# DrewSingletary/asif

Hardware: AMD Instinct MI355X
Metric: QP solves/sec (batched filter()) (higher is better)
Workload: dtype f64

## Files before the change

asif_amd/csrc/capi.hip:

```cpp
#include "asif_hip.h"
#include "launchers.hpp"
#include "multi_own.hpp"
#include <cmath>
#include <cstdlib>
#include <cstring>
#include <new>
#include <thread>
#include <vector>

using namespace asif;

struct asif_hip_ctx {
	int model, variant, device;
	asif_hip_options opts;
	asif_hip_solver solver;
	asif_hip_dims dims;
	DevOptions dev;
	double *d_in, *d_out;
	int32_t *d_rc;
	int64_t cap;
	double *s_rows;
	int64_t s_cap;
	int32_t *s_code;
	int64_t s_code_cap;
	double *s_ckpt;
	int64_t s_ckpt_cap;
	struct Realizable {
		asif_hip_realizable_options opts;
		RzDev dev;
		double *d_vertices, *d_normals, *d_facetRec, *d_table, *d_pointC;
		int32_t *d_fverts, *d_factive, *d_overflow;
	} *rz;
	struct RobustData {
		asif_hip_robust_data_options opts;
		RbDev dev;
		double *d_hp, *d_pointC;
	} *rb;
	double *d_learn;
	DevOptions::Learn learn;
	int32_t *r_rc;
	int64_t r_cap;
};

extern "C" int asif_hip_version(void) { return ASIF_HIP_VERSION; }

extern "C" const char *asif_hip_error_string(int code)
{
	switch (code) {
	case ASIF_HIP_OK: return "ok";
	case ASIF_HIP_EINVAL: return "invalid argument or unsupported model/variant pair";
	case ASIF_HIP_ENODEVICE: return "no usable HIP device (gfx950 required)";
	case ASIF_HIP_EUNSUPPORTED: return "no compiled kernel for this QP shape";
	default: return code > 0 ? hipGetErrorString((hipError_t)code) : "unknown error";
	}
}

extern "C" int asif_hip_device_count(void)
{
	int n = 0;
	if (hipGetDeviceCount(&n) != hipSuccess) return 0;
	return n;
}

extern "C" int asif_hip_default_options(int model, int variant, asif_hip_options *o)
{
	if (!o) return ASIF_HIP_EINVAL;
	std::memset(o, 0, sizeof(*o));
	o->relaxCost = 50.0;
	o->relaxLb = 5.0;
	o->relaxReachLb = 5.0;
	o->relaxTTS = 5.0;
	o->relaxMinOrtho = 5.0;
	o->backTrajHorizon = 1.0;
	o->backTrajExtend = 0.05;
	o->backTrajDt = 0.01;
	o->backTrajMinOrtho = 0.01;
	o->satSharpness = (variant == ASIF_HIP_EXPLICIT) ? 5.0 : 0.1;
	o->inf = 1e20;
	o->pMin = o->pMax = 1.0;
	o->backContDt = 0.01;
	o->n_debug = -1;
	o->npSSmax = -1;
	o->integrator = 0;
	o->backTrajAbsTol = 1.0e-6;
	o->backTrajRelTol = 1.0e-6;
	switch (model) {
	case ASIF_HIP_MODEL_DOUBLE_INTEGRATOR:
		o->lb[0] = -1.0;
		o->ub[0] = 1.0;
		break;
	case ASIF_HIP_MODEL_PLANAR_TWO_INPUT:
		o->lb[0] = o->lb[1] = -1.0;
		o->ub[0] = o->ub[1] = 1.0;
		break;
	case ASIF_HIP_MODEL_CART_PENDULUM:
		o->lb[0] = -4.0;
		o->ub[0] = 4.0;
		break;
	case ASIF_HIP_MODEL_INVERTED_PENDULUM:
		o->lb[0] = -1.5;
		o->ub[0] = 1.5;
		o->backTrajHorizon = 5.0;
		o->backTrajDt = 0.001;
		o->relaxReachLb = 5.0;
		o->relaxLb = 10.0;
		break;
	case ASIF_HIP_MODEL_SEGWAY:
		o->lb[0] = -20.0;
		o->ub[0] = 20.0;
		o->backTrajHorizon = 3.0;
		o->backTrajDt = 0.01;
		o->relaxCost = 10;
		o->relaxLb = 2.0;
		o->relaxTTS = 30.0;
		o->relaxMinOrtho = 60.0;
		o->backTrajMinOrtho = 0.001;
		break;
	case ASIF_HIP_MODEL_DOUBLE_INTEGRATOR_IMPLICIT:
		o->lb[0] = -1.0;
		o->ub[0] = 1.0;
		o->backTrajHorizon = 2.0;
		o->backTrajDt = 0.01;
		o->relaxReachLb = 5.0;
		o->relaxLb = 10.0;
		break;
	case ASIF_HIP_MODEL_DOUBLE_INTEGRATOR_TB:
		o->lb[0] = -1.0;
		o->ub[0] = 1.0;
		o->backTrajHorizon = 2.0;
		o->backTrajDt = 0.001;
		o->relaxLb = 10.0;
		o->relaxTTS = 5.0;
		o->relaxMinOrtho = 5.0;
		break;
	case ASIF_HIP_MODEL_INVERTED_PENDULUM_TB:
		o->lb[0] = -1.5;
		o->ub[0] = 1.5;
		o->backTrajHorizon = 11.0;
		o->backTrajDt = 0.001;
		o->relaxCost = 10.;
		o->relaxLb = 10.0;
		o->relaxTTS = 30.0;
		o->relaxMinOrtho = 60.0;
		o->backTrajMinOrtho = 0.001;
		break;
	case ASIF_HIP_MODEL_INVERTED_PENDULUM_ROBUST: {
		o->lb[0] = -1.5;
		o->ub[0] = 1.5;
		o->pMin = 0.8;
		o->pMax = 1.2;
		o->nHalfPlanes = 4;
		const double a = 1.0 / M_PI;
		const double hp[8] = {a, 0, -a, 0, 0, a, 0, -a};
		std::memcpy(o->halfPlanes, hp, sizeof(hp));
		break;
	}
	default:
		return ASIF_HIP_EINVAL;
	}
	return ASIF_HIP_OK;
}

extern "C" int asif_hip_default_solver(asif_hip_solver *s)
{
	if (!s) return ASIF_HIP_EINVAL;
	s->rho = 0.1;
	s->sigma = 1e-6;
	s->alpha = 1.6;
	s->eps_abs = 1e-8;
	s->eps_rel = 1e-8;
	s->eps_prim_inf = 1e-4;
	s->eps_dual_inf = 1e-4;
	s->adaptive_rho_tolerance = 5.0;
	s->max_iter = 4000;
	s->check_interval = 0;
	s->scaling_iters = 0;
	s->polish = 2;
	s->active_set_rounds = 12;
	s->refine_steps = 2;
	s->adaptive_rho = 1;
	s->lanes_per_qp = 0;
	s->presolve = 0;
	s->warm_start = 1;
	s->adaptive_rho_interval = 0;
	return ASIF_HIP_OK;
}

static double no_bound_value(double inf) { return inf > 1e30 ? 1e30 : inf; }

static int model_dims(int model, int variant, const asif_hip_options &o, asif_hip_dims &d, DevOptions &dev,
                      bool after_update = false)
{
	std::memset(&d, 0, sizeof(d));
	std::memset(&dev, 0, sizeof(dev));
// ... 448 lines not shown
	delete r;
}

static int rb_configure(asif_hip_ctx *c, const asif_hip_robust_data_options &o)
{
	asif_hip_ctx::RobustData *r = c->rb;
	RbDev &z = r->dev;
	int M = o.npSSmax;
	if (M < 0 || M > z.N) M = z.N;
	if (M < 1 || M > 8) return ASIF_HIP_EUNSUPPORTED;
	r->opts = o;
	z.npSSmax = M;
	z.relaxCost = o.relaxCost;
	z.relaxLb = o.relaxLb;
	z.inf = no_bound_value(o.inf);
	z.lb = o.lb[0];
	z.ub = o.ub[0];
	z.mMin = o.mMin;
	z.mMax = o.mMax;
	z.Klo = o.Klo;
	z.Khi = o.Khi;
	z.Flo = o.Flo;
	z.Fhi = o.Fhi;
	asif_hip_dims &d = c->dims;
	std::memset(&d, 0, sizeof(d));
	d.nx = 2;
	d.nu = 1;
	d.npSS = z.N;
	d.nv = 2 + 4 * M;
	d.nc = 3 * M;
	d.nrelax = 1;
	d.ndiag = M + 1;
	int rc = launch_robust_data_point(z, r->d_pointC, nullptr);
	if (rc) return rc;
	double pc[kRbPoint];
	hipError_t e = hipMemcpy(pc, r->d_pointC, sizeof(pc), hipMemcpyDeviceToHost);
	if (e != hipSuccess) return (int)e;
	return pc[kRbPoint - 1] != 0.0 ? ASIF_HIP_EUNSUPPORTED : ASIF_HIP_OK;
}

extern "C" int asif_hip_create_robust_data(asif_hip_ctx **out, int model, const double *halfPlanes, int32_t N,
                                           const asif_hip_robust_data_options *opts, const asif_hip_solver *solver,
                                           int device)
{
	if (!out) return ASIF_HIP_EINVAL;
	*out = nullptr;
	if (model != ASIF_HIP_MODEL_DOUBLE_INTEGRATOR_ROBUST || !halfPlanes || N < 1) return ASIF_HIP_EINVAL;
	asif_hip_robust_data_options o;
	if (opts) o = *opts;
	else asif_hip_default_robust_data_options(model, &o);
	int r = check_device(device);
	if (r) return r;
	hipError_t e = hipSetDevice(device);
	if (e != hipSuccess) return (int)e;
	asif_hip_ctx *c = new (std::nothrow) asif_hip_ctx();
	if (!c) return ASIF_HIP_EINVAL;
	std::memset(c, 0, sizeof(*c));
	c->model = model;
	c->variant = ASIF_HIP_ROBUST;
	c->device = device;
	if (solver) c->solver = *solver;
	else asif_hip_default_solver(&c->solver);
	c->rb = new (std::nothrow) asif_hip_ctx::RobustData();
	if (!c->rb) {
		delete c;
		return ASIF_HIP_EINVAL;
	}
	std::memset(c->rb, 0, sizeof(*c->rb));
	c->rb->dev.N = N;
	e = hipMalloc((void **)&c->rb->d_hp, sizeof(double) * 2 * N);
	if (e == hipSuccess) e = hipMalloc((void **)&c->rb->d_pointC, sizeof(double) * kRbPoint);
	if (e == hipSuccess) e = hipMemcpy(c->rb->d_hp, halfPlanes, sizeof(double) * 2 * N, hipMemcpyHostToDevice);
	c->rb->dev.hp = c->rb->d_hp;
	c->rb->dev.pointC = c->rb->d_pointC;
	r = (e == hipSuccess) ? rb_configure(c, o) : (int)e;
	if (r != ASIF_HIP_OK) {
		rb_free(c->rb);
		delete c;
		return r;
	}
	*out = c;
	return ASIF_HIP_OK;
}

extern "C" int asif_hip_update_robust_data_options(asif_hip_ctx *ctx, const asif_hip_robust_data_options *opts)
{
	if (!ctx || !opts || !ctx->rb) return ASIF_HIP_EINVAL;
	hipError_t e = hipSetDevice(ctx->device);
	if (e != hipSuccess) return (int)e;
	const asif_hip_robust_data_options keep = ctx->rb->opts;
	int r = rb_configure(ctx, *opts);
	if (r) (void)rb_configure(ctx, keep);
	return r;
}

extern "C" int asif_hip_destroy(asif_hip_ctx *ctx)
{
	if (!ctx) return ASIF_HIP_EINVAL;
	if (ctx->rz) {
		(void)hipSetDevice(ctx->device);
		rz_free(ctx->rz);
	}
	if (ctx->rb) {
		(void)hipSetDevice(ctx->device);
		rb_free(ctx->rb);
	}
	if (ctx->d_learn) {
		(void)hipSetDevice(ctx->device);
		(void)hipFree(ctx->d_learn);
	}
	if (ctx->r_rc) {
		(void)hipSetDevice(ctx->device);
		(void)hipFree(ctx->r_rc);
	}
	if (ctx->s_rows) {
		(void)hipSetDevice(ctx->device);
		(void)hipFree(ctx->s_rows);
	}
	if (ctx->s_code) {
		(void)hipSetDevice(ctx->device);
		(void)hipFree(ctx->s_code);
	}
	if (ctx->s_ckpt) {
		(void)hipSetDevice(ctx->device);
		(void)hipFree(ctx->s_ckpt);
	}
	if (ctx->d_in) {
		(void)hipSetDevice(ctx->device);
		(void)hipFree(ctx->d_in);
		(void)hipFree(ctx->d_out);
		(void)hipFree(ctx->d_rc);
	}
	delete ctx;
	return ASIF_HIP_OK;
}

extern "C" int asif_hip_get_dims(const asif_hip_ctx *ctx, asif_hip_dims *d)
{
	if (!ctx || !d) return ASIF_HIP_EINVAL;
	*d = ctx->dims;
	return ASIF_HIP_OK;
}

extern "C" int asif_hip_update_options(asif_hip_ctx *ctx, const asif_hip_options *opts)
{
	if (!ctx || !opts) return ASIF_HIP_EINVAL;
	asif_hip_dims d;
	DevOptions dev;
	int r = model_dims(ctx->model, ctx->variant, *opts, d, dev, true);
	if (r) return r;
	ctx->opts = *opts;
	ctx->dims = d;
	ctx->dev = dev;
	return ASIF_HIP_OK;
}

static int stage_rows(asif_hip_ctx *ctx, FilterArgs &a)
{
	const int64_t nA = (int64_t)ctx->dims.nc * ctx->dims.nv, nb = ctx->dims.nc;
	const int64_t need = (nA + nb) * a.ld;
	if (need > ctx->s_cap) {
		if (ctx->s_rows) (void)hipFree(ctx->s_rows);
		ctx->s_rows = nullptr;
		ctx->s_cap = 0;
		hipError_t e = hipMalloc((void **)&ctx->s_rows, sizeof(double) * need);
		if (e != hipSuccess) return (int)e;
		ctx->s_cap = need;
	}
	if (a.B > ctx->s_code_cap) {
		if (ctx->s_code) (void)hipFree(ctx->s_code);
		ctx->s_code = nullptr;
		ctx->s_code_cap = 0;
		hipError_t e = hipMalloc((void **)&ctx->s_code, sizeof(int32_t) * a.B);
		if (e != hipSuccess) return (int)e;
		ctx->s_code_cap = a.B;
	}
	a.A = ctx->s_rows;
	a.b = ctx->s_rows + nA * a.ld;
	a.code = ctx->s_code;
	return 0;
}

static int stage_ckpt(asif_hip_ctx *ctx, FilterArgs &a)
{
	const int64_t nz = ctx->dims.nx + ctx->dims.nx * ctx->dims.nx;
	int64_t need;
	switch (ctx->model) {
	case ASIF_HIP_MODEL_INVERTED_PENDULUM:
	case ASIF_HIP_MODEL_DOUBLE_INTEGRATOR_IMPLICIT:
	case ASIF_HIP_MODEL_INVERTED_PENDULUM_TB:
	case ASIF_HIP_MODEL_DOUBLE_INTEGRATOR_TB:
	case ASIF_HIP_MODEL_SEGWAY: need = (int64_t)ctx->dims.npBTSS * (nz + 2) * a.ld; break;
	default: return ASIF_HIP_EINVAL;
	}
	if (need > ctx->s_ckpt_cap) {
		if (ctx->s_ckpt) (void)hipFree(ctx->s_ckpt);
		ctx->s_ckpt = nullptr;
		ctx->s_ckpt_cap = 0;
		hipError_t e = hipMalloc((void **)&ctx->s_ckpt, sizeof(double) * need);
		if (e != hipSuccess) return (int)e;
		ctx->s_ckpt_cap = need;
	}
	a.ckpt = ctx->s_ckpt;
	return 0;
}

static int run_filter(asif_hip_ctx *ctx, FilterArgs a, bool assemble_only, hipStream_t stream)
{
	if (ctx->variant == ASIF_HIP_REALIZABLE)
		return ctx->rz ? launch_realizable(ctx->rz->dev, ctx->solver, a, assemble_only, stream) : ASIF_HIP_EINVAL;
	if (ctx->rb) return launch_robust_data(ctx->rb->dev, ctx->solver, a, assemble_only, stream);
	if (ctx->model == ASIF_HIP_MODEL_DOUBLE_INTEGRATOR && ctx->variant == ASIF_HIP_EXPLICIT)
		return launch_explicit_di(ctx->dev, ctx->solver, a, assemble_only, stream);
	if (ctx->model == ASIF_HIP_MODEL_PLANAR_TWO_INPUT && ctx->variant == ASIF_HIP_EXPLICIT)
		return launch_explicit_p2(ctx->dev, ctx->solver, a, assemble_only, stream);
	if (ctx->model == ASIF_HIP_MODEL_CART_PENDULUM && ctx->variant == ASIF_HIP_EXPLICIT)
		return launch_explicit_cp(ctx->dev, ctx->solver, a, assemble_only, stream);
	if (ctx->variant == ASIF_HIP_IMPLICIT_RB || (ctx->variant == ASIF_HIP_IMPLICIT && ctx->dev.useLearning)) {
		DevOptions dev = ctx->dev;
		if (dev.useLearning) {
			if (!ctx->d_learn) return ASIF_HIP_EINVAL;
			dev.learn = ctx->learn;
		}
		if (!assemble_only) {
			int r = stage_rows(ctx, a);
			if (r) return r;
		}
		if (int r = stage_ckpt(ctx, a)) return r;
		if (ctx->model == ASIF_HIP_MODEL_INVERTED_PENDULUM)
			return launch_implicit_ip(dev, ctx->solver, a, assemble_only, stream, true);
		if (ctx->model == ASIF_HIP_MODEL_DOUBLE_INTEGRATOR_IMPLICIT)
			return launch_implicit_di(dev, ctx->solver, a, assemble_only, stream, true);
		return ASIF_HIP_EINVAL;
	}
	if (ctx->model == ASIF_HIP_MODEL_INVERTED_PENDULUM && ctx->variant == ASIF_HIP_IMPLICIT) {
		if (!assemble_only) {
			int r = stage_rows(ctx, a);
			if (r) return r;
		}
		if (int r = stage_ckpt(ctx, a)) return r;
		return launch_implicit_ip(ctx->dev, ctx->solver, a, assemble_only, stream);
	}
	if (ctx->model == ASIF_HIP_MODEL_SEGWAY && ctx->variant == ASIF_HIP_IMPLICIT_TB) {
		if (!assemble_only) {
			int r = stage_rows(ctx, a);
			if (r) return r;
		}
		if (int r = stage_ckpt(ctx, a)) return r;
		return launch_tb_segway(ctx->dev, ctx->solver, a, assemble_only, stream);
	}
	if (ctx->model == ASIF_HIP_MODEL_DOUBLE_INTEGRATOR_IMPLICIT && ctx->variant == ASIF_HIP_IMPLICIT) {
		if (!assemble_only) {
			int r = stage_rows(ctx, a);
			if (r) return r;
		}
		if (int r = stage_ckpt(ctx, a)) return r;
		return launch_implicit_di(ctx->dev, ctx->solver, a, assemble_only, stream);
	}
	if (ctx->model == ASIF_HIP_MODEL_INVERTED_PENDULUM_TB && ctx->variant == ASIF_HIP_IMPLICIT_TB) {
		if (!assemble_only) {
			int r = stage_rows(ctx, a);
			if (r) return r;
		}
		if (int r = stage_ckpt(ctx, a)) return r;
		return launch_tb_pendulum(ctx->dev, ctx->solver, a, assemble_only, stream);
	}
	if (ctx->model == ASIF_HIP_MODEL_DOUBLE_INTEGRATOR_TB && ctx->variant == ASIF_HIP_IMPLICIT_TB) {
		if (!assemble_only) {
			int r = stage_rows(ctx, a);
			if (r) return r;
		}
		if (int r = stage_ckpt(ctx, a)) return r;
		return launch_tb_di(ctx->dev, ctx->solver, a, assemble_only, stream);
	}
	if (ctx->model == ASIF_HIP_MODEL_INVERTED_PENDULUM_ROBUST && ctx->variant == ASIF_HIP_ROBUST)
		return launch_robust_ip(ctx->dev, ctx->solver, a, assemble_only, stream);
	return ASIF_HIP_EINVAL;
}

extern "C" int asif_hip_filter_batch(asif_hip_ctx *ctx, int64_t B, int64_t ldx, const double *x, const double *udes,
                                     double *uact, double *relax, int32_t *rc, double *diag, void *stream)
{
	if (!ctx || B < 0 || ldx < B || (B > 0 && (!x || !udes || !uact || !relax || !rc))) return ASIF_HIP_EINVAL;
	if (B == 0) return ASIF_HIP_OK;
	hipError_t e = hipSetDevice(ctx->device);
	if (e != hipSuccess) return (int)e;
	FilterArgs a = {B, ldx, x, udes, uact, relax, rc, diag, ctx->dims.ndiag, nullptr, nullptr, nullptr};
	return run_filter(ctx, a, false, (hipStream_t)stream);
}

extern "C" int asif_hip_filter_batch_lie(asif_hip_ctx *ctx, int64_t B, int64_t ldx, const double *x, const double *udes,
                                         const double *lfh, const double *lgh, double *uact, double *relax, int32_t *rc,
                                         double *diag, void *stream)
{
	if (!ctx || B < 0 || ldx < B || (B > 0 && (!x || !udes || !lfh || !lgh || !uact || !relax || !rc)))
		return ASIF_HIP_EINVAL;
	if (ctx->variant != ASIF_HIP_EXPLICIT || ctx->rz || ctx->rb) return ASIF_HIP_EINVAL;
	if (B == 0) return ASIF_HIP_OK;
	hipError_t e = hipSetDevice(ctx->device);
	if (e != hipSuccess) return (int)e;
	FilterArgs a = {B, ldx, x, udes, uact, relax, rc, diag, ctx->dims.ndiag, nullptr, nullptr, nullptr, nullptr, lfh, lgh};
	return run_filter(ctx, a, false, (hipStream_t)stream);
}

static bool default_solver_mode(const asif_hip_solver &S, bool presolve_too = false)
{
	const bool light = S.polish == 2 || (presolve_too && S.presolve);
	return light && (S.lanes_per_qp == 0 || S.lanes_per_qp == 1);
}

extern "C" int asif_hip_filter_vjp_batch(asif_hip_ctx *ctx, int64_t B, int64_t ldx, const double *x, const double *udes,
                                         const double *lfh, const double *lgh, const double *guact, double *gudes,
                                         double *glfh, double *glgh, double *gx, int32_t *rc, void *stream)
{
	if (!ctx || B < 0 || ldx < B || (B > 0 && (!x || !udes || !guact || !gudes || !rc))) return ASIF_HIP_EINVAL;
	if ((lfh == nullptr) != (lgh == nullptr)) return ASIF_HIP_EINVAL;
	if (!lfh && (glfh || glgh || gx)) return ASIF_HIP_EINVAL;
	if (ctx->variant != ASIF_HIP_EXPLICIT || ctx->rz || ctx->rb) return ASIF_HIP_EUNSUPPORTED;
	if (!default_solver_mode(ctx->solver)) return ASIF_HIP_EUNSUPPORTED;
	if (B == 0) return ASIF_HIP_OK;
	hipError_t e = hipSetDevice(ctx->device);
	if (e != hipSuccess) return (int)e;
	const VjpArgs a = {B, ldx, x, udes, lfh, lgh, guact, gudes, glfh, glgh, gx, rc};
	if (ctx->model == ASIF_HIP_MODEL_DOUBLE_INTEGRATOR) return launch_explicit_vjp_di(ctx->dev, a, (hipStream_t)stream);
	if (ctx->model == ASIF_HIP_MODEL_PLANAR_TWO_INPUT) return launch_explicit_vjp_p2(ctx->dev, a, (hipStream_t)stream);
	if (ctx->model == ASIF_HIP_MODEL_CART_PENDULUM) return launch_explicit_vjp_cp(ctx->dev, a, (hipStream_t)stream);
	return ASIF_HIP_EUNSUPPORTED;
}

extern "C" int asif_hip_rollout_batch(asif_hip_ctx *ctx, int64_t B, int64_t ldx, int32_t T, double dt, double *x,
                                      const double *udes, double *uact, double *relax, int32_t *nfail, double *xlog,
                                      double *ulog, int32_t *rclog, void *stream)
{
	if (!ctx || B < 0 || ldx < B || T < 0 || (B > 0 && (!x || !udes || !uact || !relax || !nfail))) return ASIF_HIP_EINVAL;
	const bool fused = ctx->model == ASIF_HIP_MODEL_DOUBLE_INTEGRATOR && ctx->variant == ASIF_HIP_EXPLICIT;
	const bool staged = !ctx->rz && !ctx->rb &&
	                    (ctx->variant == ASIF_HIP_IMPLICIT || ctx->variant == ASIF_HIP_IMPLICIT_RB ||
	                     ctx->variant == ASIF_HIP_IMPLICIT_TB);
	if (!fused && !staged) return ASIF_HIP_EUNSUPPORTED;
	if (B == 0 || T == 0) return ASIF_HIP_OK;
	hipError_t e = hipSetDevice(ctx->device);
	if (e != hipSuccess) return (int)e;
	if (fused) {
		const RolloutArgs a = {B, ldx, T, dt, x, udes, uact, relax, nfail, xlog, ulog, rclog};
		return launch_rollout_explicit_di(ctx->dev, ctx->solver, a, (hipStream_t)stream);
	}
	hipStream_t s = (hipStream_t)stream;
	if (B > ctx->r_cap) {
		if (ctx->r_rc) (void)hipFree(ctx->r_rc);
		ctx->r_rc = nullptr;
		ctx->r_cap = 0;
		if ((e = hipMalloc((void **)&ctx->r_rc, sizeof(int32_t) * B)) != hipSuccess) return (int)e;
		ctx->r_cap = B;
	}
	if ((e = hipMemsetAsync(nfail, 0, sizeof(int32_t) * B, s)) != hipSuccess) return (int)e;
	const asif_hip_dims &d = ctx->dims;
	for (int32_t t = 0; t < T; t++) {
		FilterArgs a = {B, ldx, x, udes, uact, relax, ctx->r_rc, nullptr, d.ndiag, nullptr, nullptr, nullptr};
		int r = run_filter(ctx, a, false, s);
		if (r) return r;
		r = launch_plant_step(ctx->model, ctx->dev, B, ldx, dt, x, uact, ctx->r_rc, nfail,
		                      xlog ? xlog + (int64_t)t * d.nx * ldx : nullptr,
		                      ulog ? ulog + (int64_t)t * d.nu * ldx : nullptr, rclog ? rclog + (int64_t)t * ldx : nullptr, s);
		if (r) return r;
	}
	return ASIF_HIP_OK;
}

extern "C" int asif_hip_rollout_vjp_batch(asif_hip_ctx *ctx, int64_t B, int64_t ldx, int32_t T, double dt,
                                          const double *xlog, const double *ulog, const int32_t *rclog,
                                          const double *udes, const double *gxT, const double *guactT,
                                          const double *gxlog, const double *gulog, double *gx0, double *gudes,
                                          double *guact0, int32_t *nskip, void *stream)
{
	if (!ctx || B < 0 || ldx < B || T < 0) return ASIF_HIP_EINVAL;
	if (B > 0 && (!udes || !gxT || !gx0 || !gudes || !guact0 || !nskip)) return ASIF_HIP_EINVAL;
	if (B > 0 && T > 0 && (!xlog || !ulog || !rclog)) return ASIF_HIP_EINVAL;
	if (ctx->variant != ASIF_HIP_EXPLICIT || ctx->rz || ctx->rb || ctx->model != ASIF_HIP_MODEL_DOUBLE_INTEGRATOR)
		return ASIF_HIP_EUNSUPPORTED;
	if (!default_solver_mode(ctx->solver)) return ASIF_HIP_EUNSUPPORTED;
	if (B == 0) return ASIF_HIP_OK;
	hipError_t e = hipSetDevice(ctx->device);
	if (e != hipSuccess) return (int)e;
	const RolloutVjpArgs a = {B, ldx, T, dt, xlog, ulog, rclog, udes, gxT, guactT, gxlog, gulog, gx0, gudes, guact0, nskip};
	return launch_rollout_vjp_explicit_di(ctx->dev, a, (hipStream_t)stream);
}

static int policy_rollout_handle(const asif_hip_ctx *ctx, bool presolve_too)
{
	if (ctx->variant != ASIF_HIP_EXPLICIT || ctx->rz || ctx->rb || !is_rollout_model(ctx->model)) return ASIF_HIP_EUNSUPPORTED;
	return default_solver_mode(ctx->solver, presolve_too) ? ASIF_HIP_OK : ASIF_HIP_EUNSUPPORTED;
}

static int policy_rollout_forward(asif_hip_ctx *ctx, int64_t B, int64_t ldx, int32_t T, double dt, int32_t integrator,
                                  bool params, double *x, const double *K, const double *k, const double *v,
                                  const double *alpha, const double *lb, const double *ub, double *uact, double *relax,
                                  int32_t *nfail, double *xlog, double *ulog, int32_t *rclog, void *stream)
{
	if (!ctx || B < 0 || ldx < B || T < 0 || (B > 0 && (!x || !k || !uact || !relax || !nfail))) return ASIF_HIP_EINVAL;
	if (integrator != ASIF_HIP_PLANT_EULER && integrator != ASIF_HIP_PLANT_RK4) return ASIF_HIP_EINVAL;
	if (int r = policy_rollout_handle(ctx, true)) return r;
	if (B == 0 || T == 0) return ASIF_HIP_OK;
	hipError_t e = hipSetDevice(ctx->device);
	if (e != hipSuccess) return (int)e;
	const ParamRolloutArgs a = {{B, ldx, T, dt, x, K, k, v, uact, relax, nfail, xlog, ulog, rclog}, alpha, lb, ub};
	return launch_rollout_policy_explicit(ctx->model, integrator, params, ctx->dev, a, (hipStream_t)stream);
}

static int policy_rollout_backward(asif_hip_ctx *ctx, int64_t B, int64_t ldx, int32_t T, double dt, int32_t integrator,
                                   bool params, const double *xlog, const double *ulog, const int32_t *rclog,
                                   const double *K, const double *k, const double *v, const double *alpha,
                                   const double *lb, const double *ub, const double *gxT, const double *guactT,
                                   const double *gxlog, const double *gulog, double *gx0, double *gK, double *gk,
                                   double *gv, double *galpha, double *glb, double *gub, double *guact0, int32_t *nskip,
                                   void *stream)
{
	if (!ctx || B < 0 || ldx < B || T < 0) return ASIF_HIP_EINVAL;
	if (integrator != ASIF_HIP_PLANT_EULER && integrator != ASIF_HIP_PLANT_RK4) return ASIF_HIP_EINVAL;
	if (B > 0 && (!k || !gxT || !gx0 || !gk || !guact0 || !nskip)) return ASIF_HIP_EINVAL;
	if (B > 0 && T > 0 && (!xlog || !ulog || !rclog)) return ASIF_HIP_EINVAL;
	if ((gK && !K) || (gv && !v)) return ASIF_HIP_EINVAL;
	if ((galpha && !alpha) || (glb && !lb) || (gub && !ub)) return ASIF_HIP_EINVAL;
	if (int r = policy_rollout_handle(ctx, false)) return r;
	if (B == 0) return ASIF_HIP_OK;
	hipError_t e = hipSetDevice(ctx->device);
	if (e != hipSuccess) return (int)e;
	const ParamRolloutVjpArgs a = {{B,   ldx,    T,     dt,    xlog, ulog, rclog, K,  k,      v,
	                                gxT, guactT, gxlog, gulog, gx0,  gK,   gk,    gv, guact0, nskip},
	                               alpha, lb, ub, galpha, glb, gub};
	return launch_rollout_policy_vjp_explicit(ctx->model, integrator, params, ctx->dev, a, (hipStream_t)stream);
}

extern "C" int asif_hip_rollout_policy_batch(asif_hip_ctx *ctx, int64_t B, int64_t ldx, int32_t T, double dt, double *x,
                                             const double *K, const double *k, const double *v, double *uact,
                                             double *relax, int32_t *nfail, double *xlog, double *ulog, int32_t *rclog,
                                             void *stream)
{
	return policy_rollout_forward(ctx, B, ldx, T, dt, ASIF_HIP_PLANT_EULER, false, x, K, k, v, nullptr, nullptr, nullptr, uact,
	                              relax, nfail, xlog, ulog, rclog, stream);
}

extern "C" int asif_hip_rollout_policy_vjp_batch(asif_hip_ctx *ctx, int64_t B, int64_t ldx, int32_t T, double dt,
// ... 320 lines not shown
```

asif_amd/csrc/explicit_filter.hpp:

```cpp
#pragma once
#include <cstdint>
#include <cstdlib>
#include <type_traits>
#include "admm_small.hpp"
#include "launchers.hpp"

namespace asif {

template <class M, int G, bool PRE, bool SEL = false, bool WHOLE = false>
__device__ __forceinline__ void explicit_filter_body(const DevOptions &o, const asif_hip_solver &S, const FilterArgs &a,
                                                     bool assemble_only)
{
	constexpr int NX = M::NX, NU = M::NU, NP = M::NPSS, NV = NU + 1, NC = NP;
	constexpr int RPL = (NC + G - 1) / G;
	const int64_t tid = (int64_t)blockIdx.x * blockDim.x + threadIdx.x;
	const int g = (int)(tid % G);
	int64_t i = tid / G;
	const bool live = i < a.B;
	if (!live) i = a.B - 1;

	double x[NX], uDes[NU];
#pragma unroll
	for (int k = 0; k < NX; k++) x[k] = a.x[k * a.ld + i];
#pragma unroll
	for (int k = 0; k < NU; k++) uDes[k] = a.udes[k * a.ld + i];

	double h[NP], Dh[NP * NX], f[NX], gm[NX * NU];
	M::safetySet(o, x, h, Dh);
	M::dynamics(o, x, f, gm);
	double Lfh[NP], Lgh[NP * NU];
#pragma unroll
	for (int r = 0; r < NP; r++) {
		double s = 0.0;
#pragma unroll
		for (int k = 0; k < NX; k++) s += Dh[r + k * NP] * f[k];
		Lfh[r] = s;
#pragma unroll
		for (int j = 0; j < NU; j++) {
			double t = 0.0;
#pragma unroll
			for (int k = 0; k < NX; k++) t += Dh[r + k * NP] * gm[k + j * NX];
			Lgh[r + j * NP] = t;
		}
	}
	const int nkeep = SEL ? o.npKeep : NP;
	int pos[NP];
#pragma unroll
	for (int r = 0; r < NP; r++) pos[r] = r;
	if (SEL && nkeep < NP) {
#pragma unroll
		for (int r = 0; r < NP; r++) {
			int p = 0;
#pragma unroll
			for (int q = 0; q < NP; q++) p += (h[q] < h[r] || (h[q] == h[r] && q < r)) ? 1 : 0;
			pos[r] = p;
		}
	}
	if (SEL && a.lfh) {
#pragma unroll
		for (int r = 0; r < NP; r++) {
			const int p = pos[r] < nkeep ? pos[r] : 0;
			Lfh[r] = a.lfh[(int64_t)p * a.ld + i];
#pragma unroll
			for (int j = 0; j < NU; j++) Lgh[r + j * NP] = a.lgh[(int64_t)(p + j * nkeep) * a.ld + i];
		}
	}
	if (assemble_only) {
		if (live && g == 0) {
#pragma unroll
			for (int r = 0; r < NP; r++) {
				if (pos[r] < nkeep) {
					const int p = pos[r];
#pragma unroll
					for (int j = 0; j < NU; j++) a.A[(int64_t)(p + j * nkeep) * a.ld + i] = Lgh[r + j * NP];
					a.A[(int64_t)(p + NU * nkeep) * a.ld + i] = h[r];
					a.b[(int64_t)p * a.ld + i] = -Lfh[r];
				}
			}
			a.code[i] = 1;
			if (a.diag)
				for (int r = 0; r < NP; r++)
					if (pos[r] < nkeep) a.diag[(int64_t)pos[r] * a.ld + i] = (double)r;
		}
		return;
	}

	QpLaneData<NV, RPL> qp;
#pragma unroll
	for (int j = 0; j < NU; j++) {
		qp.Hd[j] = 1.0;
		qp.c[j] = -2.0 * uDes[j];
		qp.lb[j] = o.lb[j];
		qp.ub[j] = o.ub[j];
	}
	qp.Hd[NU] = o.relaxCost;
	qp.c[NU] = -2.0 * o.relaxCost * o.relaxLb;
	qp.lb[NU] = o.relaxLb;
	qp.ub[NU] = o.relaxLb;
#pragma unroll
	for (int k = 0; k < RPL; k++) {
#pragma unroll
		for (int j = 0; j < NV; j++) qp.A[k][j] = 0.0;
		qp.b[k] = -1e20;
		qp.eq[k] = false;
#pragma unroll
		for (int r = 0; r < NC; r++)
			if (r == g + k * G && pos[r] < nkeep) {
#pragma unroll
				for (int j = 0; j < NU; j++) qp.A[k][j] = Lgh[r + j * NP];
				qp.A[k][NU] = h[r];
				qp.b[k] = -Lfh[r];
			}
	}
	if constexpr (PRE) {
		static_assert(NU == 1 && G == 1, "one input: the pinned relaxation variable leaves a one-variable problem");
		double sol[NV];
		int steps;
		const int verdict = GiSmall<NV, RPL, G>::template solve_with_pinned<NU>(qp, g, 8 * NV + 4, sol, steps);
		if constexpr (WHOLE) {
			const bool ok = verdict == kGiOptimal;
			double u = fmin(fmax(sol[0], o.lb[0]), o.ub[0]), rl = sol[NU];
			if (__any(live & !ok)) {
				if (live & !ok) {
					u = a.uact[i];
					rl = a.relax[i];
				}
			}
			if (live) {
				a.uact[i] = u;
				a.relax[i] = rl;
				a.rc[i] = ok ? ASIF_HIP_RC_OK : ASIF_HIP_RC_QP_FAILED;
			}
		} else if (live) {
			if (verdict == kGiOptimal) {
				a.uact[i] = fmin(fmax(sol[0], o.lb[0]), o.ub[0]);
				a.relax[i] = sol[NU];
				a.rc[i] = ASIF_HIP_RC_OK;
			} else {
				a.rc[i] = ASIF_HIP_RC_QP_FAILED;
			}
		}
		if (live) {
			if (a.diag) {
				a.diag[0 * a.ld + i] = 0.0;
				a.diag[1 * a.ld + i] = 0.0;
				a.diag[(a.ndiag - 1) * a.ld + i] = 0.0;
			}
		}
		return;
	}

	AdmmSmall<NV, RPL, G> admm;
	double sol[NV];
	int status, iters;
	admm.solve(qp, S, sol, status, iters, false, S.polish != 1);

	if (live && g == 0) {
		if (status == kStatusSolved) {
#pragma unroll
			for (int j = 0; j < NU; j++) a.uact[j * a.ld + i] = fmin(fmax(sol[j], o.lb[j]), o.ub[j]);
			a.relax[i] = sol[NU];
			a.rc[i] = ASIF_HIP_RC_OK;
		} else {
			a.rc[i] = ASIF_HIP_RC_QP_FAILED;
		}
		if (a.diag) {
			a.diag[0 * a.ld + i] = (double)admm.stat_rounds;
			a.diag[1 * a.ld + i] = (double)admm.stat_farkas;
			a.diag[(a.ndiag - 1) * a.ld + i] = (double)iters;
		}
	}
}

template <class M, int G, bool PRE, bool SEL = false>
__global__ __launch_bounds__((PRE ? 256 : 64), (G >= 2 ? 2 : 1)) void explicit_filter_kernel(DevOptions o, asif_hip_solver S, FilterArgs a,
                                                             bool assemble_only)
{
	explicit_filter_body<M, G, PRE, SEL>(o, S, a, assemble_only);
}

template <class M, int G>
static int launch_g(const DevOptions &o, const asif_hip_solver &S0, const FilterArgs &a, bool assemble_only,
                    hipStream_t stream)
{
	const int block = 64;
	const asif_hip_solver S = resolve_scaling(S0, 1, 1);
	const bool sel = o.npKeep < M::NPSS || a.lfh != nullptr;
	if (sel)
		hipLaunchKernelGGL((explicit_filter_kernel<M, G, false, true>), dim3(grid_for(a.B, G, block)), dim3(block), 0,
		                   stream, o, S, a, assemble_only);
	else
		hipLaunchKernelGGL((explicit_filter_kernel<M, G, false, false>), dim3(grid_for(a.B, G, block)), dim3(block), 0,
		                   stream, o, S, a, assemble_only);
	return (int)hipGetLastError();
}

}
```

asif_amd/csrc/k_explicit.hip:

```cpp
#include <cstdint>
#include <cstdlib>
#include <type_traits>
#include "explicit_filter.hpp"

namespace asif {

constexpr long long kWholeLinesFrom = 6291456;
struct ExplicitOpts {
	double lb[ASIF_HIP_MAX_NU], ub[ASIF_HIP_MAX_NU], relaxCost, relaxLb;
	int npKeep;
};
template <class M, bool SEL, bool WHOLE = false>
__global__ __launch_bounds__(256) void explicit_light_kernel(ExplicitOpts e, FilterArgs a)
{
	static_assert(M::kIgnoresOptions, "the model's functors must not read DevOptions: only the class's fields are passed");
	DevOptions o = {};
#pragma unroll
	for (int j = 0; j < ASIF_HIP_MAX_NU; j++) {
		o.lb[j] = e.lb[j];
		o.ub[j] = e.ub[j];
	}
	o.relaxCost = e.relaxCost;
	o.relaxLb = e.relaxLb;
	o.npKeep = e.npKeep;
	const asif_hip_solver none = {};
	explicit_filter_body<M, 1, true, SEL, WHOLE>(o, none, a, false);
}

template <class M, bool LIGHT = false>
__global__ __launch_bounds__(LIGHT ? 256 : 64) void explicit_rollout_kernel(DevOptions o, asif_hip_solver S, RolloutArgs a)
{
	constexpr int NX = M::NX, NU = M::NU, NP = M::NPSS, NV = NU + 1, NC = NP;
	int64_t i = (int64_t)blockIdx.x * blockDim.x + threadIdx.x;
	const bool live = i < a.B;
	if (!live) i = a.B - 1;
	const int64_t ld = a.ld;
	double x[NX], uDes[NU], uAct[NU], relax;
#pragma unroll
	for (int k = 0; k < NX; k++) x[k] = a.x[k * ld + i];
#pragma unroll
	for (int k = 0; k < NU; k++) {
		uDes[k] = a.udes[k * ld + i];
		uAct[k] = a.uact[k * ld + i];
	}
	relax = a.relax[i];
	int nfail = 0;
	std::conditional_t<LIGHT, int, AdmmSmall<NV, NC, 1>> admm{};
#pragma unroll 1
	for (int t = 0; t < a.T; t++) {
		double h[NP], Dh[NP * NX], f[NX], gm[NX * NU];
		M::safetySet(o, x, h, Dh);
		M::dynamics(o, x, f, gm);
		QpLaneData<NV, NC> qp;
#pragma unroll
		for (int r = 0; r < NP; r++) {
			double s = 0.0;
#pragma unroll
			for (int k = 0; k < NX; k++) s += Dh[r + k * NP] * f[k];
#pragma unroll
			for (int j = 0; j < NU; j++) {
				double tt = 0.0;
#pragma unroll
				for (int k = 0; k < NX; k++) tt += Dh[r + k * NP] * gm[k + j * NX];
				qp.A[r][j] = tt;
			}
			qp.A[r][NU] = h[r];
			qp.b[r] = -s;
			qp.eq[r] = false;
		}
		if (o.npKeep < NP) {
#pragma unroll
			for (int r = 0; r < NP; r++) {
				int p = 0;
#pragma unroll
				for (int q = 0; q < NP; q++) p += (h[q] < h[r] || (h[q] == h[r] && q < r)) ? 1 : 0;
				const bool kept = p < o.npKeep;
#pragma unroll
				for (int j = 0; j < NV; j++) qp.A[r][j] = kept ? qp.A[r][j] : 0.0;
				qp.b[r] = kept ? qp.b[r] : -1e20;
			}
		}
#pragma unroll
		for (int j = 0; j < NU; j++) {
			qp.Hd[j] = 1.0;
			qp.c[j] = -2.0 * uDes[j];
			qp.lb[j] = o.lb[j];
			qp.ub[j] = o.ub[j];
		}
		qp.Hd[NU] = o.relaxCost;
		qp.c[NU] = -2.0 * o.relaxCost * o.relaxLb;
		qp.lb[NU] = o.relaxLb;
		qp.ub[NU] = o.relaxLb;
		double sol[NV];
		int status, iters;
		if constexpr (LIGHT) {
			static_assert(NU == 1, "one input: the pinned relaxation variable leaves a one-variable problem");
			const int verdict = GiSmall<NV, NC, 1>::template solve_with_pinned<NU>(qp, 0, 8 * NV + 4, sol, iters);
			status = verdict == kGiOptimal ? kStatusSolved : kStatusPrimalInf;
		} else {
			admm.solve(qp, S, sol, status, iters, S.warm_start != 0 && t > 0, S.polish != 1);
		}
		if (live && a.xlog) {
#pragma unroll
			for (int k = 0; k < NX; k++) a.xlog[((int64_t)t * NX + k) * ld + i] = x[k];
		}
		const bool ok = status == kStatusSolved;
		if (ok) {
#pragma unroll
			for (int j = 0; j < NU; j++) uAct[j] = fmin(fmax(sol[j], o.lb[j]), o.ub[j]);
			relax = sol[NU];
		} else nfail++;
		if (live && a.ulog) {
#pragma unroll
			for (int j = 0; j < NU; j++) a.ulog[((int64_t)t * NU + j) * ld + i] = uAct[j];
		}
		if (live && a.rclog) a.rclog[(int64_t)t * ld + i] = ok ? ASIF_HIP_RC_OK : ASIF_HIP_RC_QP_FAILED;
		{
#pragma clang fp contract(off)
#pragma unroll
			for (int k = 0; k < NX; k++) {
				double fcl = 0.0;
				fcl += f[k];
#pragma unroll
				for (int j = 0; j < NU; j++) fcl += uAct[j] * gm[k + j * NX];
				x[k] += a.dt * fcl;
			}
		}
	}
	if (!live) return;
#pragma unroll
	for (int k = 0; k < NX; k++) a.x[k * ld + i] = x[k];
#pragma unroll
	for (int j = 0; j < NU; j++) a.uact[j * ld + i] = uAct[j];
	a.relax[i] = relax;
	a.nfail[i] = nfail;
}

int launch_rollout_explicit_di(const DevOptions &o, const asif_hip_solver &S0, const RolloutArgs &a, hipStream_t stream)
{
	if (a.B <= 0 || a.T <= 0) return 0;
	const asif_hip_solver S = resolve_scaling(S0, 1, 1);
	if (S.polish == 2 || S.presolve)
		hipLaunchKernelGGL((explicit_rollout_kernel<DoubleIntegrator, true>), dim3(grid_for(a.B, 1, 256)), dim3(256), 0,
		                   stream, o, S, a);
	else
		hipLaunchKernelGGL((explicit_rollout_kernel<DoubleIntegrator, false>), dim3(grid_for(a.B, 1, 64)), dim3(64), 0,
		                   stream, o, S, a);
	return (int)hipGetLastError();
}

int launch_explicit_di(const DevOptions &o, const asif_hip_solver &S, const FilterArgs &a, bool assemble_only,
                       hipStream_t stream)
{
	if (a.B <= 0) return 0;
	if ((S.presolve || (S.polish == 2 && (S.lanes_per_qp == 0 || S.lanes_per_qp == 1))) && !assemble_only) {
		const int block = 256;
		const bool sel = o.npKeep < DoubleIntegrator::NPSS || a.lfh != nullptr;
		ExplicitOpts e;
		for (int j = 0; j < ASIF_HIP_MAX_NU; j++) {
			e.lb[j] = o.lb[j];
			e.ub[j] = o.ub[j];
		}
		e.relaxCost = o.relaxCost;
		e.relaxLb = o.relaxLb;
		e.npKeep = o.npKeep;
		static const int64_t whole_from = []() {
			const char *v = getenv("ASIF_HIP_WHOLE_LINES_FROM");
			return v ? (int64_t)atoll(v) : (int64_t)kWholeLinesFrom;
		}();
		if (!sel && a.B >= whole_from) {
			hipLaunchKernelGGL((explicit_light_kernel<DoubleIntegrator, false, true>), dim3(grid_for(a.B, 1, block)), dim3(block), 0,
			                   stream, e, a);
			return (int)hipGetLastError();
		}
		if (sel)
			hipLaunchKernelGGL((explicit_light_kernel<DoubleIntegrator, true>), dim3(grid_for(a.B, 1, block)), dim3(block), 0,
			                   stream, e, a);
		else
			hipLaunchKernelGGL((explicit_light_kernel<DoubleIntegrator, false>), dim3(grid_for(a.B, 1, block)), dim3(block), 0,
			                   stream, e, a);
		return (int)hipGetLastError();
	}
	switch (S.lanes_per_qp) {
	case 2: return launch_g<DoubleIntegrator, 2>(o, S, a, assemble_only, stream);
	case 4: return launch_g<DoubleIntegrator, 4>(o, S, a, assemble_only, stream);
	case 0:
	case 1: return launch_g<DoubleIntegrator, 1>(o, S, a, assemble_only, stream);
	default: return ASIF_HIP_EINVAL;
	}
}

int launch_explicit_p2(const DevOptions &o, const asif_hip_solver &S, const FilterArgs &a, bool assemble_only,
                       hipStream_t stream)
{
	if (a.B <= 0) return 0;
	if (S.lanes_per_qp > 1) return ASIF_HIP_EINVAL;
	return launch_g<PlanarTwoInput, 1>(o, S, a, assemble_only, stream);
}

}
```

asif_amd/csrc/launchers.hpp:

```cpp
#pragma once
#include <cstdlib>
#include <hip/hip_runtime.h>
#include <stdint.h>
#include "asif_hip.h"
#include "models.hpp"

namespace asif {

struct FilterArgs {
	int64_t B, ld;
	const double *x, *udes;
	double *uact, *relax;
	int32_t *rc;
	double *diag;
	int ndiag;
	double *A, *b;
	int32_t *code;
	double *ckpt;
	const double *lfh, *lgh;
	int compactRows;
	int fuseQp;
};

int launch_explicit_di(const DevOptions &o, const asif_hip_solver &S, const FilterArgs &a, bool assemble_only,
                       hipStream_t stream);
int launch_explicit_p2(const DevOptions &o, const asif_hip_solver &S, const FilterArgs &a, bool assemble_only,
                       hipStream_t stream);
int launch_explicit_cp(const DevOptions &o, const asif_hip_solver &S, const FilterArgs &a, bool assemble_only,
                       hipStream_t stream);

struct VjpArgs {
	int64_t B, ld;
	const double *x, *udes, *lfh, *lgh;
	const double *guact;
	double *gudes;
	double *glfh, *glgh, *gx;
	int32_t *rc;
};
int launch_explicit_vjp_di(const DevOptions &o, const VjpArgs &a, hipStream_t stream);
int launch_explicit_vjp_p2(const DevOptions &o, const VjpArgs &a, hipStream_t stream);
int launch_explicit_vjp_cp(const DevOptions &o, const VjpArgs &a, hipStream_t stream);

struct RolloutArgs {
	int64_t B, ld;
	int T;
	double dt;
	double *x;
	const double *udes;
	double *uact;
	double *relax;
	int32_t *nfail;
	double *xlog;
	double *ulog;
	int32_t *rclog;
};
int launch_rollout_explicit_di(const DevOptions &o, const asif_hip_solver &S, const RolloutArgs &a, hipStream_t stream);
struct RolloutVjpArgs {
	int64_t B, ld;
	int T;
	double dt;
	const double *xlog, *ulog;
	const int32_t *rclog;
	const double *udes;
	const double *gxT;
	const double *guactT;
	const double *gxlog;
	const double *gulog;
	double *gx0, *gudes, *guact0;
	int32_t *nskip;
};
int launch_rollout_vjp_explicit_di(const DevOptions &o, const RolloutVjpArgs &a, hipStream_t stream);
struct PolicyRolloutArgs {
	int64_t B, ld;
	int T;
	double dt;
	double *x;
	const double *K, *k, *v;
	double *uact, *relax;
	int32_t *nfail;
	double *xlog, *ulog;
	int32_t *rclog;
};
struct PolicyRolloutVjpArgs {
	int64_t B, ld;
	int T;
	double dt;
	const double *xlog, *ulog;
	const int32_t *rclog;
	const double *K, *k, *v;
	const double *gxT, *guactT, *gxlog, *gulog;
	double *gx0, *gK, *gk, *gv, *guact0;
	int32_t *nskip;
};
struct ParamRolloutArgs {
	PolicyRolloutArgs p;
	const double *alpha, *lb, *ub;
};
struct ParamRolloutVjpArgs {
	PolicyRolloutVjpArgs p;
	const double *alpha, *lb, *ub;
	double *galpha, *glb, *gub;
};
template <class F>
int with_rollout_model(int model, F &&f)
{
	switch (model) {
	case ASIF_HIP_MODEL_DOUBLE_INTEGRATOR: return f(DoubleIntegrator{});
	case ASIF_HIP_MODEL_CART_PENDULUM: return f(CartPendulum{});
	default: return ASIF_HIP_EUNSUPPORTED;
	}
}
inline bool is_rollout_model(int model)
{
	return with_rollout_model(model, [](auto) { return 0; }) == 0;
}
int launch_rollout_policy_explicit(int model, int integrator, bool params, const DevOptions &o, const ParamRolloutArgs &a,
                                   hipStream_t stream);
int launch_rollout_policy_vjp_explicit(int model, int integrator, bool params, const DevOptions &o,
                                       const ParamRolloutVjpArgs &a, hipStream_t stream);
int launch_plant_step(int model, const DevOptions &o, int64_t B, int64_t ld, double dt, double *x, const double *uact,
                      const int32_t *rc, int32_t *nfail, double *xlog, double *ulog, int32_t *rclog, hipStream_t s);

int launch_implicit_ip(const DevOptions &o, const asif_hip_solver &S, const FilterArgs &a, bool assemble_only,
                       hipStream_t stream, bool rb = false);

int launch_implicit_di(const DevOptions &o, const asif_hip_solver &S, const FilterArgs &a, bool assemble_only,
                       hipStream_t stream, bool rb = false);

int launch_tb_segway(const DevOptions &o, const asif_hip_solver &S, const FilterArgs &a, bool assemble_only,
                     hipStream_t stream);

int launch_tb_pendulum(const DevOptions &o, const asif_hip_solver &S, const FilterArgs &a, bool assemble_only,
                       hipStream_t stream);

int launch_tb_di(const DevOptions &o, const asif_hip_solver &S, const FilterArgs &a, bool assemble_only, hipStream_t stream);

int launch_robust_ip(const DevOptions &o, const asif_hip_solver &S, const FilterArgs &a, bool assemble_only,
                     hipStream_t stream);

constexpr int kRzRec = 12;
constexpr int kRzPoint = 8;
struct RzDev {
	const double *facetRec;
	const double *table;
	const double *pointC;
	int nF, nA, maxCrit, npSSmax, npSS, nv, nc;
	double unc[2];
	double relaxDes, relaxOffset, relaxCost, inf, lb, ub;
	double mMin, mMax, Klo, Khi, Flo, Fhi;
};
int launch_realizable_tables(const RzDev &z, const double *vertices, const int32_t *fverts, const double *normals,
                             const int32_t *factive, double *facetRec, double *table, double *pointC,
                             int32_t *overflow, hipStream_t stream);
int launch_realizable(const RzDev &z, const asif_hip_solver &S, const FilterArgs &a, bool assemble_only,
                      hipStream_t stream);

constexpr int kRbPoint = 12;
struct RbDev {
	const double *hp;
	const double *pointC;
	int N, npSSmax;
	double relaxCost, relaxLb, inf, lb, ub;
	double mMin, mMax, Klo, Khi, Flo, Fhi;
};
int launch_robust_data_point(const RbDev &z, double *pointC, hipStream_t stream);
int launch_robust_data(const RbDev &z, const asif_hip_solver &S, const FilterArgs &a, bool assemble_only,
                       hipStream_t stream);

constexpr int kXcds = 8;
__host__ __device__ inline unsigned xcd_grid(int64_t B) { return (unsigned)(kXcds * ((B + kXcds - 1) / kXcds)); }
__device__ __forceinline__ int64_t xcd_contiguous_index(unsigned block, int64_t B)
{
	const int64_t per = (B + kXcds - 1) / kXcds;
	return (int64_t)(block % kXcds) * per + block / kXcds;
}

struct QpArgs {
	int64_t B, ld;
	int nv, nc;
	const double *Hd, *c, *A, *b, *lb, *ub;
	uint64_t be_mask;
	double *sol;
	int32_t *status, *iters;
// ... 65 lines not shown
```

Measured before the change: 19.33 billion.

## Add prepared light-path launch with cached function handles and 32-bit indexing

```diff
diff --git a/asif_amd/csrc/capi.hip b/asif_amd/csrc/capi.hip
--- a/asif_amd/csrc/capi.hip
+++ b/asif_amd/csrc/capi.hip
@@ -40,6 +40,7 @@
 	DevOptions::Learn learn;
 	int32_t *r_rc;
 	int64_t r_cap;
+	PreparedLight light;
 };
 
 extern "C" int asif_hip_version(void) { return ASIF_HIP_VERSION; }
@@ -794,6 +795,7 @@
 	ctx->opts = *opts;
 	ctx->dims = d;
 	ctx->dev = dev;
+	ctx->light.state = PreparedLight::kUnset;
 	return ASIF_HIP_OK;
 }
 
@@ -925,11 +927,26 @@
 {
 	if (!ctx || B < 0 || ldx < B || (B > 0 && (!x || !udes || !uact || !relax || !rc))) return ASIF_HIP_EINVAL;
 	if (B == 0) return ASIF_HIP_OK;
-	hipError_t e = hipSetDevice(ctx->device);
-	if (e != hipSuccess) return (int)e;
+	int current = -1;
+	hipError_t e = hipGetDevice(&current);
+	if (e != hipSuccess || current != ctx->device) e = hipSetDevice(ctx->device);
+	if (e != hipSuccess) return (int)e;
+	PreparedLight &p = ctx->light;
+	if (p.state == PreparedLight::kUnset) {
+		if (ctx->model == ASIF_HIP_MODEL_DOUBLE_INTEGRATOR && ctx->variant == ASIF_HIP_EXPLICIT && !ctx->rz && !ctx->rb) {
+			if (int r = prepare_explicit_light_di(ctx->dev, ctx->solver, ctx->dims.ndiag, p)) return r;
+		} else {
+			p.state = PreparedLight::kGeneral;
+		}
+	}
+	if (p.state == PreparedLight::kReady && B < p.whole_from)
+		return launch_prepared_light(p, B, ldx, x, udes, uact, relax, rc, diag, (hipStream_t)stream);
 	FilterArgs a = {B, ldx, x, udes, uact, relax, rc, diag, ctx->dims.ndiag, nullptr, nullptr, nullptr};
 	return run_filter(ctx, a, false, (hipStream_t)stream);
 }
+
+extern "C" int asif_test_explicit_light_index32(int64_t ld) { return explicit_light_index32(ld, DoubleIntegrator::NX) ? 1 : 0; }
+extern "C" int asif_test_prepared_state(const asif_hip_ctx *ctx) { return ctx ? ctx->light.state : ASIF_HIP_EINVAL; }
 
 extern "C" int asif_hip_filter_batch_lie(asif_hip_ctx *ctx, int64_t B, int64_t ldx, const double *x, const double *udes,
                                          const double *lfh, const double *lgh, double *uact, double *relax, int32_t *rc,
diff --git a/asif_amd/csrc/explicit_filter.hpp b/asif_amd/csrc/explicit_filter.hpp
--- a/asif_amd/csrc/explicit_filter.hpp
+++ b/asif_amd/csrc/explicit_filter.hpp
@@ -7,15 +7,16 @@
 
 namespace asif {
 
-template <class M, int G, bool PRE, bool SEL = false, bool WHOLE = false>
-__device__ __forceinline__ void explicit_filter_body(const DevOptions &o, const asif_hip_solver &S, const FilterArgs &a,
+template <class M, int G, bool PRE, bool SEL = false, bool WHOLE = false, class Args = FilterArgs>
+__device__ __forceinline__ void explicit_filter_body(const DevOptions &o, const asif_hip_solver &S, const Args &a,
                                                      bool assemble_only)
 {
 	constexpr int NX = M::NX, NU = M::NU, NP = M::NPSS, NV = NU + 1, NC = NP;
 	constexpr int RPL = (NC + G - 1) / G;
-	const int64_t tid = (int64_t)blockIdx.x * blockDim.x + threadIdx.x;
+	using I = typename Args::index_t;
+	const I tid = (I)blockIdx.x * blockDim.x + threadIdx.x;
 	const int g = (int)(tid % G);
-	int64_t i = tid / G;
+	I i = tid / G;
 	const bool live = i < a.B;
 	if (!live) i = a.B - 1;
 
@@ -56,33 +57,37 @@
 			pos[r] = p;
 		}
 	}
-	if (SEL && a.lfh) {
-#pragma unroll
-		for (int r = 0; r < NP; r++) {
-			const int p = pos[r] < nkeep ? pos[r] : 0;
-			Lfh[r] = a.lfh[(int64_t)p * a.ld + i];
-#pragma unroll
-			for (int j = 0; j < NU; j++) Lgh[r + j * NP] = a.lgh[(int64_t)(p + j * nkeep) * a.ld + i];
-		}
-	}
-	if (assemble_only) {
-		if (live && g == 0) {
+	if constexpr (SEL) {
+		if (a.lfh) {
 #pragma unroll
 			for (int r = 0; r < NP; r++) {
-				if (pos[r] < nkeep) {
-					const int p = pos[r];
-#pragma unroll
-					for (int j = 0; j < NU; j++) a.A[(int64_t)(p + j * nkeep) * a.ld + i] = Lgh[r + j * NP];
-					a.A[(int64_t)(p + NU * nkeep) * a.ld + i] = h[r];
-					a.b[(int64_t)p * a.ld + i] = -Lfh[r];
+				const int p = pos[r] < nkeep ? pos[r] : 0;
+				Lfh[r] = a.lfh[(int64_t)p * a.ld + i];
+#pragma unroll
+				for (int j = 0; j < NU; j++) Lgh[r + j * NP] = a.lgh[(int64_t)(p + j * nkeep) * a.ld + i];
+			}
+		}
+	}
+	if constexpr (!PRE) {
+		if (assemble_only) {
+			if (live && g == 0) {
+#pragma unroll
+				for (int r = 0; r < NP; r++) {
+					if (pos[r] < nkeep) {
+						const int p = pos[r];
+#pragma unroll
+						for (int j = 0; j < NU; j++) a.A[(int64_t)(p + j * nkeep) * a.ld + i] = Lgh[r + j * NP];
+						a.A[(int64_t)(p + NU * nkeep) * a.ld + i] = h[r];
+						a.b[(int64_t)p * a.ld + i] = -Lfh[r];
+					}
 				}
-			}
-			a.code[i] = 1;
-			if (a.diag)
-				for (int r = 0; r < NP; r++)
-					if (pos[r] < nkeep) a.diag[(int64_t)pos[r] * a.ld + i] = (double)r;
-		}
-		return;
+				a.code[i] = 1;
+				if (a.diag)
+					for (int r = 0; r < NP; r++)
+						if (pos[r] < nkeep) a.diag[(int64_t)pos[r] * a.ld + i] = (double)r;
+			}
+			return;
+		}
 	}
 
 	QpLaneData<NV, RPL> qp;
@@ -142,9 +147,9 @@
 		}
 		if (live) {
 			if (a.diag) {
-				a.diag[0 * a.ld + i] = 0.0;
-				a.diag[1 * a.ld + i] = 0.0;
-				a.diag[(a.ndiag - 1) * a.ld + i] = 0.0;
+				a.diag[i] = 0.0;
+				a.diag[(int64_t)a.ld + i] = 0.0;
+				a.diag[(int64_t)(a.ndiag - 1) * a.ld + i] = 0.0;
 			}
 		}
 		return;
diff --git a/asif_amd/csrc/explicit_light_args.hpp b/asif_amd/csrc/explicit_light_args.hpp
--- /dev/null
+++ b/asif_amd/csrc/explicit_light_args.hpp
@@ -0,0 +1,27 @@
+#pragma once
+#include <cstddef>
+#include <stdint.h>
+
+namespace asif {
+
+struct ExplicitLightArgs {
+	int64_t B, ld;
+	const double *x, *udes;
+	double *uact, *relax;
+	int32_t *rc;
+	double *diag;
+	double lb, ub, relaxCost, relaxLb;
+	int32_t ndiag;
+};
+static_assert(offsetof(ExplicitLightArgs, B) == 0 && offsetof(ExplicitLightArgs, ld) == 8 && offsetof(ExplicitLightArgs, x) == 16 &&
+                  offsetof(ExplicitLightArgs, udes) == 24 && offsetof(ExplicitLightArgs, uact) == 32 &&
+                  offsetof(ExplicitLightArgs, relax) == 40 && offsetof(ExplicitLightArgs, rc) == 48 &&
+                  offsetof(ExplicitLightArgs, diag) == 56 && offsetof(ExplicitLightArgs, lb) == 64 &&
+                  offsetof(ExplicitLightArgs, ub) == 72 && offsetof(ExplicitLightArgs, relaxCost) == 80 &&
+                  offsetof(ExplicitLightArgs, relaxLb) == 88 && offsetof(ExplicitLightArgs, ndiag) == 96,
+              "the block is packed without holes: host and device compilers must agree on every offset");
+static_assert(sizeof(ExplicitLightArgs) == 104 && sizeof(ExplicitLightArgs) <= 128, "one argument block of at most 128 bytes");
+
+constexpr bool explicit_light_index32(int64_t ld, int nx) { return ld >= 0 && ld <= (int64_t)INT32_MAX / nx; }
+
+}
diff --git a/asif_amd/csrc/k_explicit.hip b/asif_amd/csrc/k_explicit.hip
--- a/asif_amd/csrc/k_explicit.hip
+++ b/asif_amd/csrc/k_explicit.hip
@@ -25,6 +25,75 @@
 	o.npKeep = e.npKeep;
 	const asif_hip_solver none = {};
 	explicit_filter_body<M, 1, true, SEL, WHOLE>(o, none, a, false);
+}
+
+template <class I>
+struct LightView {
+	using index_t = I;
+	I B, ld;
+	const double *x, *udes;
+	double *uact, *relax;
+	int32_t *rc;
+	double *diag;
+	int ndiag;
+};
+template <class M, class I>
+__global__ __launch_bounds__(256) void explicit_light_kernel_flat(ExplicitLightArgs k)
+{
+	static_assert(M::kIgnoresOptions && M::NU == 1, "one input, functors that do not read DevOptions");
+	DevOptions o = {};
+	o.lb[0] = k.lb;
+	o.ub[0] = k.ub;
+	o.relaxCost = k.relaxCost;
+	o.relaxLb = k.relaxLb;
+	o.npKeep = M::NPSS;
+	const LightView<I> a = {(I)k.B, (I)k.ld, k.x, k.udes, k.uact, k.relax, k.rc, k.diag, k.ndiag};
+	const asif_hip_solver none = {};
+	explicit_filter_body<M, 1, true, false, false>(o, none, a, false);
+}
+
+static int64_t whole_lines_from()
+{
+	static const int64_t v = []() {
+		const char *e = getenv("ASIF_HIP_WHOLE_LINES_FROM");
+		return e ? (int64_t)atoll(e) : (int64_t)kWholeLinesFrom;
+	}();
+	return v;
+}
+
+static unsigned light_block()
+{
+	static const unsigned v = []() {
+		const char *e = getenv("ASIF_HIP_LIGHT_BLOCK");
+		const int b = e ? atoi(e) : 0;
+		return (b == 64 || b == 128 || b == 256) ? (unsigned)b : 256u;
+	}();
+	return v;
+}
+
+static bool light_mode(const asif_hip_solver &S)
+{
+	return S.presolve || (S.polish == 2 && (S.lanes_per_qp == 0 || S.lanes_per_qp == 1));
+}
+
+int prepare_explicit_light_di(const DevOptions &o, const asif_hip_solver &S, int ndiag, PreparedLight &p)
+{
+	p.state = PreparedLight::kGeneral;
+	if (!light_mode(S) || o.npKeep < DoubleIntegrator::NPSS) return 0;
+	hipError_t e = hipGetFuncBySymbol(&p.fn[0], (const void *)explicit_light_kernel_flat<DoubleIntegrator, int64_t>);
+	if (e == hipSuccess)
+		e = hipGetFuncBySymbol(&p.fn[1], (const void *)explicit_light_kernel_flat<DoubleIntegrator, int32_t>);
+	if (e != hipSuccess) return (int)e;
+	p.blk = {};
+	p.blk.lb = o.lb[0];
+	p.blk.ub = o.ub[0];
+	p.blk.relaxCost = o.relaxCost;
+	p.blk.relaxLb = o.relaxLb;
+	p.blk.ndiag = ndiag;
+	p.whole_from = whole_lines_from();
+	p.block = light_block();
+	p.state = PreparedLight::kReady;
+	return 0;
 }
 
 template <class M, bool LIGHT = false>
@@ -153,9 +222,15 @@
                        hipStream_t stream)
 {
 	if (a.B <= 0) return 0;
-	if ((S.presolve || (S.polish == 2 && (S.lanes_per_qp == 0 || S.lanes_per_qp == 1))) && !assemble_only) {
+	if (light_mode(S) && !assemble_only) {
 		const int block = 256;
 		const bool sel = o.npKeep < DoubleIntegrator::NPSS || a.lfh != nullptr;
+		const int64_t whole_from = whole_lines_from();
+		if (!sel && a.B < whole_from) {
+			PreparedLight p;
+			if (int r = prepare_explicit_light_di(o, S, a.ndiag, p)) return r;
+			return launch_prepared_light(p, a.B, a.ld, a.x, a.udes, a.uact, a.relax, a.rc, a.diag, stream);
+		}
 		ExplicitOpts e;
 		for (int j = 0; j < ASIF_HIP_MAX_NU; j++) {
 			e.lb[j] = o.lb[j];
@@ -164,20 +239,11 @@
 		e.relaxCost = o.relaxCost;
 		e.relaxLb = o.relaxLb;
 		e.npKeep = o.npKeep;
-		static const int64_t whole_from = []() {
-			const char *v = getenv("ASIF_HIP_WHOLE_LINES_FROM");
-			return v ? (int64_t)atoll(v) : (int64_t)kWholeLinesFrom;
-		}();
-		if (!sel && a.B >= whole_from) {
+		if (!sel)
 			hipLaunchKernelGGL((explicit_light_kernel<DoubleIntegrator, false, true>), dim3(grid_for(a.B, 1, block)), dim3(block), 0,
 			                   stream, e, a);
-			return (int)hipGetLastError();
-		}
-		if (sel)
+		else
 			hipLaunchKernelGGL((explicit_light_kernel<DoubleIntegrator, true>), dim3(grid_for(a.B, 1, block)), dim3(block), 0,
-			                   stream, e, a);
-		else
-			hipLaunchKernelGGL((explicit_light_kernel<DoubleIntegrator, false>), dim3(grid_for(a.B, 1, block)), dim3(block), 0,
 			                   stream, e, a);
 		return (int)hipGetLastError();
 	}
diff --git a/asif_amd/csrc/launchers.hpp b/asif_amd/csrc/launchers.hpp
--- a/asif_amd/csrc/launchers.hpp
+++ b/asif_amd/csrc/launchers.hpp
@@ -3,11 +3,13 @@
 #include <hip/hip_runtime.h>
 #include <stdint.h>
 #include "asif_hip.h"
+#include "explicit_light_args.hpp"
 #include "models.hpp"
 
 namespace asif {
 
 struct FilterArgs {
+	using index_t = int64_t;
 	int64_t B, ld;
 	const double *x, *udes;
 	double *uact, *relax;
@@ -29,6 +31,34 @@
 int launch_explicit_cp(const DevOptions &o, const asif_hip_solver &S, const FilterArgs &a, bool assemble_only,
                        hipStream_t stream);
 
+struct PreparedLight {
+	enum { kUnset = 0, kReady = 1, kGeneral = 2 };
+	int state;
+	hipFunction_t fn[2];
+	ExplicitLightArgs blk;
+	int64_t whole_from;
+	unsigned block;
+};
+int prepare_explicit_light_di(const DevOptions &o, const asif_hip_solver &S, int ndiag, PreparedLight &p);
+inline int launch_prepared_light(const PreparedLight &p, int64_t B, int64_t ld, const double *x, const double *udes,
+                                 double *uact, double *relax, int32_t *rc, double *diag, hipStream_t stream)
+{
+	ExplicitLightArgs k = p.blk;
+	k.B = B;
+	k.ld = ld;
+	k.x = x;
+	k.udes = udes;
+	k.uact = uact;
+	k.relax = relax;
+	k.rc = rc;
+	k.diag = diag;
+	size_t size = sizeof(k);
+	void *extra[] = {HIP_LAUNCH_PARAM_BUFFER_POINTER, &k, HIP_LAUNCH_PARAM_BUFFER_SIZE, &size, HIP_LAUNCH_PARAM_END};
+	const unsigned grid = (unsigned)((B + p.block - 1) / p.block);
+	return (int)hipModuleLaunchKernel(p.fn[explicit_light_index32(ld, DoubleIntegrator::NX) ? 1 : 0], grid, 1, 1, p.block, 1, 1, 0,
+	                                  stream, nullptr, extra);
+}
+
 struct VjpArgs {
 	int64_t B, ld;
 	const double *x, *udes, *lfh, *lgh;
```

After: 20.89 billion, median of 6. 8.1% higher.
